# PickNikRobotics/pick_ik

Measured on AMD Instinct MI355X. Metric: converged IK solves/sec (7-DOF Panda, batched random targets), higher is better.
Workload: dtype f64; 1 GPU; panda 7-DOF memetic IK (BASELINE configs[1]): population 128, elites 4, batch 4096 random reachable targets per GPU per step, seed = ready pose, max_generations 100, gd_max_iters 25; robot=panda, dof=7, tip_frames=1, batch_per_gpu=4096, batches_per_call=64, calls=21, streams=4, problems_in_flight_per_gpu=1048576, parallelism=shard1, arithmetic=exact

## Files before the change

### pick_ik_amd/csrc/pik_amd.hip

```cpp
#include <hip/hip_runtime.h>

#include <chrono>
#include <cmath>
#include <cstdlib>
#include <memory>
#include <new>
#include <string>
#include <thread>
#include <vector>

#include "pik_cartesian_ops.hpp"
#include "pik_globalpath_ops.hpp"
#include "pik_interp.hpp"
#include "pik_path_ops.hpp"
#include "pik_polyline_ops.hpp"
#include "pik_restart_ops.hpp"
#include "pik_route_ops.hpp"
#include "pik_search_ops.hpp"
#include "pik_solver.hpp"
#include "pik_startpath_ops.hpp"
#include "pik_urdf.hpp"
#include "pik_pathvalid_ops.hpp"
#include "pik_validity_ops.hpp"

namespace pik {
char* error_buffer() {
    static thread_local char buf[ERROR_BUFFER_SIZE] = "";
    return buf;
}
}

using pik::fail;

#if !defined(PIK_STRICT)
namespace pik_exact {
char* error_buffer() { return ::pik::error_buffer(); }
PIK_DECLARE_OPS_FAMILY(void, launch)
PIK_DECLARE_OPS_FAMILY(void, path)
PIK_DECLARE_OPS_FAMILY(void, search)
PIK_DECLARE_OPS_FAMILY(void, route)
PIK_DECLARE_OPS_FAMILY(void, restart)
PIK_DECLARE_OPS_FAMILY(void, startpath)
PIK_DECLARE_OPS_FAMILY(void, globalpath)
PIK_DECLARE_OPS_FAMILY(void, cartesian)
PIK_DECLARE_OPS_FAMILY(void, polyline)
PIK_DECLARE_OPS_FAMILY(void, validity)
PIK_DECLARE_OPS_FAMILY(void, pathvalid)
}
namespace pik_common {
char* error_buffer() { return ::pik::error_buffer(); }
PIK_DECLARE_OPS_FAMILY(void, launch)
PIK_DECLARE_OPS_FAMILY(void, route)
PIK_DECLARE_OPS_FAMILY(void, restart)
}
namespace pik_common_goals {
char* error_buffer() { return ::pik::error_buffer(); }
PIK_DECLARE_OPS_FAMILY(void, launch)
PIK_DECLARE_OPS_FAMILY(void, route)
PIK_DECLARE_OPS_FAMILY(void, restart)
}
#endif

namespace {

enum Flavour {
    FL_HOME,
#if !defined(PIK_STRICT)
    FL_EXACT,
    FL_COMMON,
    FL_COMMON_GOALS,
#endif
    N_FLAVOURS
};
enum Family { FAM_LAUNCH, FAM_PATH, FAM_SEARCH, FAM_ROUTE, FAM_RESTART, FAM_STARTPATH, FAM_GLOBALPATH, FAM_CARTESIAN, FAM_POLYLINE, FAM_VALIDITY, FAM_PATHVALID, N_FAMILIES };

struct SolverExt : pikamd_solver {
    int search_schedule = pik::SEARCH_ADAPTIVE;
    pik::DevBuf search_rows[pik::N_SLOTS];
    int device_regime = 1;
    long long regime_threshold = 0;
    int routed_passes[pik::N_SLOTS];
    pik::DevBuf restart_rows[pik::N_SLOTS];
    bool gate_set = false;
    pikamd_gate gate = {0.0, 0.0};
    pik::DevBuf gate_params_dev;
    pik::ParamsK gate_params_host[pik::N_SLOTS];
    bool gate_params_valid[pik::N_SLOTS] = {};
    pik::DevBuf startpath_rows[pik::N_SLOTS];
    pik::DevBuf globalpath_rows[pik::N_SLOTS];
    pik::DevBuf cartesian_goals[pik::N_SLOTS];
    pik::DevBuf polyline_rows[pik::N_SLOTS];
    bool validity_set = false;
    pik::ValidityModelK validity_model;
    pik::DevBuf validity_dev;
    uint32_t planar_xy_mask = 0;
    int path_validity = 0;
    pik::DevBuf pathvalid_rows[pik::N_SLOTS];
    SolverExt() {
        for (int& v : routed_passes) v = -1;
    }
};
SolverExt* ext_of(pikamd_solver* s) { return static_cast<SolverExt*>(s); }
const SolverExt* ext_of(const pikamd_solver* s) { return static_cast<const SolverExt*>(s); }

using OpsLookup = const void* (*)(int dof);
template <class Ops, const Ops* (*lookup)(int)>
const void* untyped(int dof) {
    return lookup(dof);
}
const OpsLookup OPS_TABLE[N_FLAVOURS][N_FAMILIES] = {
    {untyped<pik::LaunchOps, pik::launch_ops>, untyped<pik::PathOps, pik::path_ops>, untyped<pik::SearchOps, pik::search_ops>,
#if defined(PIK_STRICT)
     nullptr,
#else
     untyped<pik::RouteOps, pik::route_ops>,
#endif
     untyped<pik::RestartOps, pik::restart_ops>, untyped<pik::StartPathOps, pik::startpath_ops>,
     untyped<pik::GlobalPathOps, pik::globalpath_ops>, untyped<pik::CartesianOps, pik::cartesian_ops>,
     untyped<pik::PolylineOps, pik::polyline_ops>,
#if defined(PIK_STRICT)
     untyped<pik::ValidityOps, pik::validity_ops>, untyped<pik::PathValidOps, pik::pathvalid_ops>},
#else
     nullptr, nullptr},
    {pik_exact::launch_ops, pik_exact::path_ops, pik_exact::search_ops, pik_exact::route_ops, pik_exact::restart_ops,
     pik_exact::startpath_ops, pik_exact::globalpath_ops, pik_exact::cartesian_ops, pik_exact::polyline_ops,
     pik_exact::validity_ops, pik_exact::pathvalid_ops},
    {pik_common::launch_ops, nullptr, nullptr, pik_common::route_ops, pik_common::restart_ops, nullptr, nullptr, nullptr, nullptr, nullptr, nullptr},
    {pik_common_goals::launch_ops, nullptr, nullptr, pik_common_goals::route_ops, pik_common_goals::restart_ops, nullptr, nullptr, nullptr, nullptr, nullptr, nullptr},
#endif
};
const char* const FLAVOUR_NAMESPACE[N_FLAVOURS] = {
#if defined(PIK_STRICT)
    "pik_strict",
#else
    "pik", "pik_exact", "pik_common", "pik_common_goals",
#endif
};

template <class Ops>
const Ops* ops_at(Flavour f, Family family, int dof) {
    const OpsLookup lookup = OPS_TABLE[f][family];
    return lookup ? static_cast<const Ops*>(lookup(dof)) : nullptr;
}

int check_solver(const pikamd_solver* s) {
    if (!s) return fail(PIKAMD_EINVAL, "solver handle is NULL");
    return 0;
}

[[maybe_unused]] bool needs_literal(const pikamd_solver* s) {
    bool f = s->opt.exact || s->chain.float_mask != 0u || s->chain.n_mimic != 0;
    for (int k = 1; k < s->n_tips; ++k) f = f || s->more[k - 1].float_mask != 0u || s->more[k - 1].n_mimic != 0;
    return f;
}
[[maybe_unused]] bool needs_literal(const pikamd_solver* s, const pikamd_params* p) {
    return needs_literal(s) || (p && p->gd_step_size > 1.0e-2);
}

[[maybe_unused]] bool common_eligible(const pikamd_solver* s, const pikamd_params* p, const pik::ParamsK& pk) {
    if (!s->opt.specialised || needs_literal(s)) return false;
    const uint32_t all = (s->chain.dof >= 32) ? ~0u : ((1u << s->chain.dof) - 1u);
    auto chain_ok = [&](const pik::ChainHost& c) {
        return c.prismatic_mask == 0u && c.dh_general_mask == 0u && c.bounded_mask == all;
    };
    if (!chain_ok(s->chain)) return false;
    for (int k = 1; k < s->n_tips; ++k)
        if (!chain_ok(s->more[k - 1])) return false;
    if (pk.line_delta == 0 || !(pk.pos_scale > 0.0) || !(pk.rot_scale > 0.0)) return false;
    if (p->mode == 0 && (pk.elites != 4 || p->memetic_num_threads > 1)) return false;
    return true;
}

Flavour flavour_of(const pikamd_solver* s, const pikamd_params* p, const pik::ParamsK* pk) {
#if defined(PIK_STRICT)
    (void)s, (void)p, (void)pk;
    return FL_HOME;
#else
    if (pk && common_eligible(s, p, *pk)) return pk->goal_mask != 0 ? FL_COMMON_GOALS : FL_COMMON;
    return needs_literal(s, p) ? FL_EXACT : FL_HOME;
#endif
}
bool is_common(Flavour f) {
#if defined(PIK_STRICT)
    (void)f;
    return false;
#else
    return f == FL_COMMON || f == FL_COMMON_GOALS;
#endif
}
Flavour unspecialised(Flavour f) { return is_common(f) ? FL_HOME : f; }
bool is_exact(Flavour f) { return pik::EXACT_FLAVOUR || (f != FL_HOME && !is_common(f)); }

const pik::LaunchOps* ops_of(const pikamd_solver* s, const pikamd_params* p = nullptr) {
    return ops_at<pik::LaunchOps>(flavour_of(s, p, nullptr), FAM_LAUNCH, s->chain.dof);
}
const pik::LaunchOps* solve_ops_of(const pikamd_solver* s, const pikamd_params* p, const pik::ParamsK& pk) {
    const Flavour f = flavour_of(s, p, &pk);
    if (const pik::LaunchOps* o = ops_at<pik::LaunchOps>(f, FAM_LAUNCH, s->chain.dof)) return o;
    return ops_at<pik::LaunchOps>(unspecialised(f), FAM_LAUNCH, s->chain.dof);
}

const pik::RouteOps* route_ops_of(const pikamd_solver* s, const pikamd_params* p, const pik::ParamsK& pk) {
    const pik::SolverOptions& o = s->opt;
    if (!ext_of(s)->device_regime || p->mode != 0 || s->n_tips != 1 || p->memetic_num_threads > 1 || o.lpe != 0 ||
        o.n_sched != 0 || o.regime != 0)
        return nullptr;
    return ops_at<pik::RouteOps>(flavour_of(s, p, &pk), FAM_ROUTE, s->chain.dof);
}

int run_solve(pikamd_solver* s, const pikamd_params* p, const pik::ParamsK& pk, pik::BatchRecord* rec, int n,
              unsigned long long rng_seed, hipStream_t stream, int slot) {
    SolverExt* x = ext_of(s);
    if (const pik::RouteOps* r = route_ops_of(s, p, pk)) {
        pik::RouteCtx ctx;
        ctx.threshold = x->regime_threshold;
        if (int rc = r->solve(s, p, pk, rec, n, rng_seed, stream, slot, &ctx)) return rc;
        if (ctx.served) {
            x->routed_passes[slot] = ctx.n_passes;
            return 0;
        }
    }
    x->routed_passes[slot] = -1;
    return solve_ops_of(s, p, pk)->solve(s, p, pk, rec, n, rng_seed, stream, slot, false);
}

int no_kernels(int dof) {
    return fail(PIKAMD_EUNSUPPORTED, "dof %d: kernels are instantiated for 1..16", dof);
}

const pik::PathOps* path_ops_of(const pikamd_solver* s, const pikamd_params* p) {
    return ops_at<pik::PathOps>(flavour_of(s, p, nullptr), FAM_PATH, s->chain.dof);
}
const pik::SearchOps* search_ops_of(const pikamd_solver* s, const pikamd_params* p) {
    return ops_at<pik::SearchOps>(flavour_of(s, p, nullptr), FAM_SEARCH, s->chain.dof);
}
const pik::StartPathOps* startpath_ops_of(const pikamd_solver* s, const pikamd_params* p) {
    return ops_at<pik::StartPathOps>(flavour_of(s, p, nullptr), FAM_STARTPATH, s->chain.dof);
}
const pik::GlobalPathOps* globalpath_ops_of(const pikamd_solver* s, const pikamd_params* p) {
    return ops_at<pik::GlobalPathOps>(flavour_of(s, p, nullptr), FAM_GLOBALPATH, s->chain.dof);
}
const pik::RestartOps* restart_ops_of(const pikamd_solver* s, const pikamd_params* p, const pik::ParamsK& pk) {
    return ops_at<pik::RestartOps>(flavour_of(s, p, &pk), FAM_RESTART, s->chain.dof);
}

size_t align8(size_t v) { return (v + 7) & ~(size_t)7; }

constexpr size_t GATE_PARAMS_STRIDE = 256;
static_assert(sizeof(pik::ParamsK) <= GATE_PARAMS_STRIDE, "gate parameters slot too small");
int gate_for_call(pikamd_solver* s, const pik::ParamsK& pk, int slot, hipStream_t st, int* on, double* joint,
                  const pik::ParamsK** dev) {
    SolverExt* x = ext_of(s);
    *on = (x->gate_set && pk.approx) ? 1 : 0;
    *joint = x->gate.joint_threshold;
    *dev = nullptr;
    if (!*on) return 0;
    if (int rc = x->gate_params_dev.ensure(GATE_PARAMS_STRIDE * (size_t)pik::N_SLOTS)) return rc;
    char* d = (char*)x->gate_params_dev.p + GATE_PARAMS_STRIDE * (size_t)slot;
    const pik::ParamsK want = pik::gate_params_k(pk, x->gate.cost_threshold);
    if (!x->gate_params_valid[slot] || std::memcmp(&x->gate_params_host[slot], &want, sizeof want) != 0) {
        if (s->consts_valid[slot]) HIP_TRY(hipStreamSynchronize(s->consts_stream[slot]));
        x->gate_params_valid[slot] = false;
        std::memcpy(&x->gate_params_host[slot], &want, sizeof want);
        HIP_TRY(hipMemcpyAsync(d, &x->gate_params_host[slot], sizeof want, hipMemcpyHostToDevice, st));
        HIP_TRY(hipStreamSynchronize(st));
        x->gate_params_valid[slot] = true;
    }
    *dev = reinterpret_cast<const pik::ParamsK*>(d);
    return 0;
}

const pik::ValidityOps* validity_ops_of(const pikamd_solver* s) {
#if defined(PIK_STRICT)
    return ops_at<pik::ValidityOps>(FL_HOME, FAM_VALIDITY, s->chain.dof);
#else
    return ops_at<pik::ValidityOps>(FL_EXACT, FAM_VALIDITY, s->chain.dof);
#endif
}

int validity_chain_ok(const pikamd_solver* s, const char* who) {
    if (s->n_tips != 1) return fail(PIKAMD_EUNSUPPORTED, "%s: the validity model is for handles with one tip frame", who);
    if ((s->chain.float_mask | s->chain.skip_mask) != 0u)
        return fail(PIKAMD_EUNSUPPORTED, "%s: the validity model does not know floating joints", who);
    if (s->chain.n_mimic != 0) return fail(PIKAMD_EUNSUPPORTED, "%s: the validity model does not know mimic joints", who);
    return 0;
}

int validity_for_call(pikamd_solver* s, const char* who, const pik::ValidityOps** ops) {
    *ops = nullptr;
    if (!ext_of(s)->validity_set) return 0;
    if (int rc = validity_chain_ok(s, who)) return rc;
    *ops = validity_ops_of(s);
    return *ops ? 0 : no_kernels(s->chain.dof);
}

int path_validity_for_call(pikamd_solver* s, const char* who, const pik::PathValidOps** ops) {
    *ops = nullptr;
    if (!ext_of(s)->path_validity || !ext_of(s)->validity_set) return 0;
    if (int rc = validity_chain_ok(s, who)) return rc;
#if defined(PIK_STRICT)
    *ops = ops_at<pik::PathValidOps>(FL_HOME, FAM_PATHVALID, s->chain.dof);
#else
    *ops = ops_at<pik::PathValidOps>(FL_EXACT, FAM_PATHVALID, s->chain.dof);
#endif
    return *ops ? 0 : no_kernels(s->chain.dof);
}

int path_validity_reached(pikamd_solver* s, int slot, int64_t P, int32_t* callers, int32_t** out) {
    *out = callers;
    if (callers) return 0;
    pik::DevBuf& buf = ext_of(s)->pathvalid_rows[slot];
// ... 119 lines not shown
    if (int rc = pikamd_urdf_extract(urdf_xml, base_link, tip_links, n_tips, m.get())) return rc;
    if (m->n_tips == 1) {
        const auto& t = m->tips[0];
        pikamd_chain c{m->dof, &t.origin_xyz_rpy[0][0], &t.axis[0][0], t.joint_type, t.tip_xyz_rpy,
                       m->qmin,  m->qmax,               m->vmax,       m->bounded};
        if (int rc = pikamd_create(&c, device_ordinal, out)) return rc;
        if (m->n_mimic)
            if (int rc = pikamd_set_mimic_joints(*out, m->n_mimic, m->mimic)) {
                pikamd_destroy(*out);
                *out = nullptr;
                return rc;
            }
        return 0;
    }
    pikamd_tip tips[PIKAMD_MAX_TIPS];
    for (int k = 0; k < m->n_tips; ++k) {
        const auto& t = m->tips[k];
        tips[k] = pikamd_tip{t.n_joints, t.variable, &t.origin_xyz_rpy[0][0], &t.axis[0][0], t.joint_type, t.tip_xyz_rpy};
    }
    pikamd_multi_chain c{m->dof, m->n_tips, tips, m->qmin, m->qmax, m->vmax, m->bounded};
    if (int rc = pikamd_create_multi(&c, device_ordinal, out)) return rc;
    if (m->n_mimic)
        if (int rc = pikamd_set_mimic_joints(*out, m->n_mimic, m->mimic)) {
            pikamd_destroy(*out);
            *out = nullptr;
            return rc;
        }
    return 0;
}

int32_t pikamd_n_tips(const pikamd_solver* s) { return s ? s->n_tips : 0; }

int32_t pikamd_set_mimic_joints(pikamd_solver* s, int32_t n, const pikamd_mimic_joint* joints) {
    if (int rc = check_solver(s)) return rc;
    if (n < 0 || (n > 0 && !joints)) return fail(PIKAMD_EINVAL, "bad arguments");
    pik::ChainHost saved[PIKAMD_MAX_TIPS];
    for (int k = 0; k < s->n_tips; ++k) saved[k] = k == 0 ? s->chain : s->more[k - 1];
    auto path = [&](int k) -> pik::ChainHost& { return k == 0 ? s->chain : s->more[k - 1]; };
    for (int k = 0; k < s->n_tips; ++k) pik::clear_mimic_joints(path(k));
    for (int i = 0; i < n; ++i) {
        const pikamd_mimic_joint& m = joints[i];
        const char* msg = (m.tip < 0 || m.tip >= s->n_tips) ? "mimic joint: tip out of range" : pik::add_mimic_joint(path(m.tip), m);
        if (!msg && s->n_tips > 1) {
            const uint32_t act = path(m.tip).active_mask;
            if (!((act >> m.master_variable) & 1u) || (m.after_variable >= 0 && !((act >> m.after_variable) & 1u)))
                msg = "mimic joint: master_variable / after_variable is not on that tip's path";
        }
        if (msg) {
            for (int k = 0; k < s->n_tips; ++k) path(k) = saved[k];
            return fail(PIKAMD_EINVAL, "%s", msg);
        }
    }
    s->self_tested.clear();
    s->opt.disabled_lanes = 0;
    s->opt.disabled_lanes_exact = 0;
    return 0;
}

void pikamd_destroy(pikamd_solver* s) {
    if (!s) return;
    (void)hipSetDevice(s->device);
    (void)hipDeviceSynchronize();
    if (s->counters) (void)hipFree(s->counters);
    if (s->consts_dev) (void)hipFree(s->consts_dev);
    if (s->consts_host) (void)hipHostFree(s->consts_host);
    if (s->tables_dev) (void)hipFree(s->tables_dev);
    if (s->tables_host) (void)hipHostFree(s->tables_host);
    for (auto& ev : s->table_event)
        if (ev) (void)hipEventDestroy(ev);
    for (auto& ev : s->slot_event)
        if (ev) (void)hipEventDestroy(ev);
    for (auto& b : s->stage) b.release();
    for (auto& b : s->slot_state) b.release();
    for (auto& b : s->slot_soa) b.release();
    for (auto& b : ext_of(s)->search_rows) b.release();
    for (auto& b : ext_of(s)->restart_rows) b.release();
    for (auto& b : ext_of(s)->startpath_rows) b.release();
    for (auto& b : ext_of(s)->cartesian_goals) b.release();
    for (auto& b : ext_of(s)->polyline_rows) b.release();
    for (auto& b : ext_of(s)->globalpath_rows) b.release();
    ext_of(s)->gate_params_dev.release();
    ext_of(s)->validity_dev.release();
    for (auto& b : ext_of(s)->pathvalid_rows) b.release();
    for (auto& j : s->jobs) {
        j.dev.release();
        j.host.release();
        if (j.stream) (void)hipStreamDestroy(j.stream);
    }
    delete ext_of(s);
}

int32_t pikamd_variables(const pikamd_solver* s, double* out) {
    if (int rc = check_solver(s)) return rc;
    if (!out) return fail(PIKAMD_EINVAL, "out is NULL");
    for (int j = 0; j < s->chain.dof; ++j) {
        out[7 * j + 0] = s->chain.qmin[j];
        out[7 * j + 1] = s->chain.qmax[j];
        out[7 * j + 2] = s->chain.mid[j];
        out[7 * j + 3] = s->chain.hspan[j];
        out[7 * j + 4] = s->chain.vrcp[j];
        out[7 * j + 5] = s->chain.mdf[j];
        out[7 * j + 6] = ((s->chain.bounded_mask >> j) & 1u) ? 1.0 : 0.0;
    }
    return 0;
}

int32_t pikamd_fk_batch_device(pikamd_solver* s, int64_t n, const double* d_q, double* d_pos_quat,
                               void* stream) {
    if (int rc = check_solver(s)) return rc;
    if (n < 0 || (n > 0 && (!d_q || !d_pos_quat))) return fail(PIKAMD_EINVAL, "bad arguments");
    HIP_TRY(hipSetDevice(s->device));
    return ops_of(s)->fk(s, n, d_q, d_pos_quat, (hipStream_t)stream);
}

int32_t pikamd_fk_batch(pikamd_solver* s, int64_t n, const double* q, double* pos_quat) {
    if (int rc = check_solver(s)) return rc;
    if (n < 0 || (n > 0 && (!q || !pos_quat))) return fail(PIKAMD_EINVAL, "bad arguments");
    if (n == 0) return 0;
    HIP_TRY(hipSetDevice(s->device));
    const size_t d = (size_t)s->chain.dof;
    if (int rc = s->stage[0].ensure(sizeof(double) * d * (size_t)n)) return rc;
    if (int rc = s->stage[1].ensure(sizeof(double) * 7 * (size_t)s->n_tips * (size_t)n)) return rc;
    HIP_TRY(hipMemcpy(s->stage[0].p, q, sizeof(double) * d * (size_t)n, hipMemcpyHostToDevice));
    if (int rc = pikamd_fk_batch_device(s, n, (const double*)s->stage[0].p, (double*)s->stage[1].p, nullptr))
        return rc;
    HIP_TRY(hipMemcpy(pos_quat, s->stage[1].p, sizeof(double) * 7 * (size_t)s->n_tips * (size_t)n, hipMemcpyDeviceToHost));
    return 0;
}

int32_t pikamd_cost_batch(pikamd_solver* s, const pikamd_params* p, int64_t n,
                          const double* goal_pos_quat, const double* seed, const double* q,
                          double* cost, int32_t* is_solution) {
    if (int rc = check_solver(s)) return rc;
    pik::ParamsK pk;
    if (!p) return fail(PIKAMD_EINVAL, "params is NULL");
    if (const char* msg = pik::make_params_k(p, pk)) {
        pikamd_params q2 = *p;
        q2.mode = 1;
        if (const char* m2 = pik::make_params_k(&q2, pk)) return fail(PIKAMD_EINVAL, "%s", m2);
        (void)msg;
    }
    if (n < 0 || (n > 0 && (!goal_pos_quat || !seed || !q))) return fail(PIKAMD_EINVAL, "bad arguments");
    if (n == 0) return 0;
    HIP_TRY(hipSetDevice(s->device));
    const size_t d = (size_t)s->chain.dof, N = (size_t)n;
    if (int rc = s->stage[0].ensure(sizeof(double) * 7 * (size_t)s->n_tips * N)) return rc;
    if (int rc = s->stage[1].ensure(sizeof(double) * d * N)) return rc;
    if (int rc = s->stage[2].ensure(sizeof(double) * d * N)) return rc;
    if (int rc = s->stage[3].ensure(sizeof(double) * N)) return rc;
    if (int rc = s->stage[4].ensure(sizeof(int) * N)) return rc;
    HIP_TRY(hipMemcpy(s->stage[0].p, goal_pos_quat, sizeof(double) * 7 * (size_t)s->n_tips * N, hipMemcpyHostToDevice));
    HIP_TRY(hipMemcpy(s->stage[1].p, seed, sizeof(double) * d * N, hipMemcpyHostToDevice));
    HIP_TRY(hipMemcpy(s->stage[2].p, q, sizeof(double) * d * N, hipMemcpyHostToDevice));
    if (int rc = ops_of(s)->cost(s, pk, n, (const double*)s->stage[0].p, (const double*)s->stage[1].p,
                                 (const double*)s->stage[2].p, cost ? (double*)s->stage[3].p : nullptr,
                                 is_solution ? (int*)s->stage[4].p : nullptr, nullptr))
        return rc;
    if (cost) HIP_TRY(hipMemcpy(cost, s->stage[3].p, sizeof(double) * N, hipMemcpyDeviceToHost));
    if (is_solution) HIP_TRY(hipMemcpy(is_solution, s->stage[4].p, sizeof(int) * N, hipMemcpyDeviceToHost));
    HIP_TRY(hipDeviceSynchronize());
    return 0;
}

int32_t pikamd_gd_step_batch(pikamd_solver* s, const pikamd_params* p, int64_t n,
                             const double* goal_pos_quat, const double* seed, double* local,
                             double* best, double* local_cost, double* best_cost,
// ... 62 lines not shown
        r.stats = b.stats;
        r.completed = b.completed;
        sum += b.B;
    }
    (void)s;
    *total = sum;
    return n;
}

__global__ void pik_joint_layout_kernel(const double* __restrict__ in, double* __restrict__ out, long long B, int D,
                                        int to_aos) {
    const long long i = (long long)blockIdx.x * blockDim.x + threadIdx.x;
    if (i >= B * D) return;
    if (to_aos) {
        const long long b = i / D;
        const int j = (int)(i - b * D);
        out[i] = in[(long long)j * B + b];
    } else {
        const long long j = i / B, b = i - j * B;
        out[i] = in[b * D + j];
    }
}

static int maybe_self_test(pikamd_solver* s, const pikamd_params* p);

static int32_t solve_records(pikamd_solver* s, const pikamd_params* p, pik::BatchRecord* rec, int n,
                             uint64_t rng_seed, hipStream_t stream, int slot) {
    pik::ParamsK pk;
    if (const char* msg = pik::make_params_k(p, pk)) return fail(PIKAMD_EINVAL, "%s", msg);
    if (n == 0) return 0;
    HIP_TRY(hipSetDevice(s->device));
    if (!s->opt.soa) return run_solve(s, p, pk, rec, n, rng_seed, stream, slot);
    const int D = s->chain.dof;
    size_t doubles = 0;
    for (int k = 0; k < n; ++k) {
        if (rec[k].completed)
            return fail(PIKAMD_EINVAL, "joint_layout soa: completion counters are not available (the solutions of a "
                                       "batch are in place when the stream has passed the call)");
        doubles += (size_t)rec[k].B * (size_t)D * (rec[k].guess != rec[k].seed ? 3u : 2u);
    }
    if (int rc = s->slot_soa[slot].ensure(sizeof(double) * doubles)) return rc;
    double* w = (double*)s->slot_soa[slot].p;
    double* user_solution[PIKAMD_MAX_BATCHES];
    auto move = [&](const double* in, double* out, long long B, int to_aos) -> int {
        const long long items = B * D;
        hipLaunchKernelGGL(pik_joint_layout_kernel, dim3((unsigned)((items + 255) / 256)), dim3(256), 0, stream, in, out, B,
                           D, to_aos);
        HIP_TRY(hipGetLastError());
        return 0;
    };
    for (int k = 0; k < n; ++k) {
        const long long B = rec[k].B;
        const bool own_guess = rec[k].guess != rec[k].seed;
        double* sd = w;
        w += (size_t)B * D;
        if (int rc = move(rec[k].seed, sd, B, 1)) return rc;
        double* gs = sd;
        if (own_guess) {
            gs = w;
            w += (size_t)B * D;
            if (int rc = move(rec[k].guess, gs, B, 1)) return rc;
        }
        user_solution[k] = rec[k].solution;
        rec[k].seed = sd;
        rec[k].guess = gs;
        rec[k].solution = w;
        w += (size_t)B * D;
    }
    if (int rc = run_solve(s, p, pk, rec, n, rng_seed, stream, slot)) return rc;
    for (int k = 0; k < n; ++k)
        if (int rc = move(rec[k].solution, user_solution[k], rec[k].B, 0)) return rc;
    return 0;
}

int32_t pikamd_solve_batches_device(pikamd_solver* s, const pikamd_params* p, int32_t n_batches,
                                    const pikamd_batch* batches, uint64_t rng_seed, void* stream,
                                    int32_t slot) {
    if (int rc = check_solver(s)) return rc;
    if (slot < 0 || slot >= PIKAMD_MAX_SLOTS) return fail(PIKAMD_EINVAL, "slot out of range");
    pik::BatchRecord rec[PIKAMD_MAX_BATCHES];
    long long total = 0;
    const int n = make_records(s, n_batches, batches, rec, &total);
    if (n < 0) return n;
    return solve_records(s, p, rec, n, rng_seed, (hipStream_t)stream, slot);
}

int32_t pikamd_solve_batch_device(pikamd_solver* s, const pikamd_params* p, int64_t B,
                                  const double* d_goal_pos_quat, const double* d_seed,
                                  uint64_t rng_seed, int64_t problem_offset, double* d_solution,
                                  int32_t* d_status, double* d_final_cost, pikamd_stats* d_stats,
                                  void* stream, int32_t slot) {
    const pikamd_batch b = {B,          d_goal_pos_quat, d_seed,       nullptr, problem_offset,
                            d_solution, d_status,        d_final_cost, d_stats, nullptr};
    return pikamd_solve_batches_device(s, p, 1, &b, rng_seed, stream, slot);
}

int32_t pikamd_reserve(pikamd_solver* s, const pikamd_params* p, int64_t B, int32_t slot, void* stream) {
    if (int rc = check_solver(s)) return rc;
    pik::ParamsK pk;
    if (const char* msg = pik::make_params_k(p, pk)) return fail(PIKAMD_EINVAL, "%s", msg);
    if (B < 0) return fail(PIKAMD_EINVAL, "bad arguments");
    if (slot < 0 || slot >= PIKAMD_MAX_SLOTS) return fail(PIKAMD_EINVAL, "slot out of range");
    if (B == 0) return 0;
    if (int rc = maybe_self_test(s, p)) return rc;
    HIP_TRY(hipSetDevice(s->device));
    if (s->opt.soa)
        if (int rc = s->slot_soa[slot].ensure(sizeof(double) * (size_t)B * (size_t)s->chain.dof * 3u)) return rc;
    pik::BatchRecord rec;
    std::memset(&rec, 0, sizeof rec);
    rec.B = B;
    return solve_ops_of(s, p, pk)->solve(s, p, pk, &rec, 1, 0, (hipStream_t)stream, slot, true);
}

static int32_t start_job(pikamd_solver* s, const pikamd_params* p, int32_t n_batches,
                         const pikamd_batch* batches, uint64_t rng_seed, int job) {
    if (int rc = check_solver(s)) return rc;
    if (job < 0 || job > pik::JOB_SELF_TEST) return fail(PIKAMD_EINVAL, "job out of range");
    if (job != pik::JOB_SELF_TEST)
        if (int rc = maybe_self_test(s, p)) return rc;
    pik::HostJob& J = s->jobs[job];
    if (J.pending) return fail(PIKAMD_EINVAL, "job %d is still in flight: call pikamd_wait first", job);
    pik::BatchRecord rec[PIKAMD_MAX_BATCHES];
    long long total = 0;
    const int n = make_records(s, n_batches, batches, rec, &total);
    if (n < 0) return n;
    {
        pik::ParamsK pk;
        if (const char* msg = pik::make_params_k(p, pk)) return fail(PIKAMD_EINVAL, "%s", msg);
    }
    J.n_batches = 0;
    if (n == 0) return 0;
    HIP_TRY(hipSetDevice(s->device));
    if (!J.stream) HIP_TRY(hipStreamCreateWithFlags(&J.stream, hipStreamNonBlocking));
    const size_t d = (size_t)s->chain.dof, g7 = 7 * (size_t)s->n_tips;
    size_t off = 0;
    size_t in_goal[PIKAMD_MAX_BATCHES], in_seed[PIKAMD_MAX_BATCHES], in_guess[PIKAMD_MAX_BATCHES];
    for (int k = 0; k < n; ++k) {
        const size_t N = (size_t)rec[k].B;
        in_goal[k] = off;
        off += sizeof(double) * g7 * N;
        in_seed[k] = off;
        off += sizeof(double) * d * N;
        in_guess[k] = (rec[k].guess != rec[k].seed) ? off : in_seed[k];
        if (rec[k].guess != rec[k].seed) off += sizeof(double) * d * N;
    }
    J.in_bytes = off;
    for (int k = 0; k < n; ++k) {
        const size_t N = (size_t)rec[k].B;
        pik::HostJob::Out& o = J.outs[k];
        o.B = rec[k].B;
        o.solution = rec[k].solution;
        o.status = rec[k].status;
        o.final_cost = rec[k].cost;
        o.stats = (pikamd_stats*)rec[k].stats;
        o.off_solution = off;
        off += sizeof(double) * d * N;
        o.off_cost = off;
        off += sizeof(double) * N;
        o.off_stats = off;
        off += sizeof(pikamd_stats) * N;
        o.off_status = off;
        off += align8(sizeof(int32_t) * N);
    }
    J.out_bytes = off - J.in_bytes;
    if (int rc = J.dev.ensure(off)) return rc;
    if (int rc = J.host.ensure(off)) return rc;
    char* hb = (char*)J.host.p;
    char* db = (char*)J.dev.p;
    for (int k = 0; k < n; ++k) {
        const size_t N = (size_t)rec[k].B;
        std::memcpy(hb + in_goal[k], rec[k].goal, sizeof(double) * g7 * N);
        std::memcpy(hb + in_seed[k], rec[k].seed, sizeof(double) * d * N);
        if (in_guess[k] != in_seed[k]) std::memcpy(hb + in_guess[k], rec[k].guess, sizeof(double) * d * N);
        rec[k].goal = (const double*)(db + in_goal[k]);
        rec[k].seed = (const double*)(db + in_seed[k]);
        rec[k].guess = (const double*)(db + in_guess[k]);
        rec[k].solution = (double*)(db + J.outs[k].off_solution);
        rec[k].status = (int*)(db + J.outs[k].off_status);
        rec[k].cost = (double*)(db + J.outs[k].off_cost);
        rec[k].stats = (void*)(db + J.outs[k].off_stats);
        rec[k].completed = nullptr;
    }
    HIP_TRY(hipMemcpyAsync(db, hb, J.in_bytes, hipMemcpyHostToDevice, J.stream));
    if (int rc = solve_records(s, p, rec, n, rng_seed, J.stream, pik::N_DEVICE_SLOTS + job)) {
        (void)hipStreamSynchronize(J.stream);
        return rc;
    }
    {
// ... 119 lines not shown
        if (v != "none" && (!ints(v, ',', x) || x.size() > 15))
            return fail(PIKAMD_EINVAL, "passes: expected 'none' or up to 15 ascending generation marks, got '%s'", v.c_str());
        for (size_t k = 0; k < x.size(); ++k)
            if (x[k] <= 0 || (k > 0 && x[k] <= x[k - 1]))
                return fail(PIKAMD_EINVAL, "passes: marks must be positive and ascending, got '%s'", v.c_str());
        o.passes_set = true;
        o.n_marks = (int)x.size();
        for (size_t k = 0; k < x.size(); ++k) o.marks[k] = x[k];
        return 0;
    }
    if (n == "two_per_simd") {
        if (v.empty()) { o.two_per_simd = -1; return 0; }
        std::vector<int> x;
        if (!ints(v, ',', x) || x.size() != 1 || x[0] < 0)
            return fail(PIKAMD_EINVAL, "two_per_simd: expected 0, 1 or a wavefront threshold, got '%s'", v.c_str());
        o.two_per_simd = x[0];
        return 0;
    }
    if (n == "arithmetic") {
#if defined(PIK_STRICT)
        if (v.empty() || v == "exact") return 0;
        return fail(PIKAMD_EINVAL, "arithmetic: the verification library only has 'exact', got '%s'", v.c_str());
#else
        if (v.empty() || v == "exact") { o.exact = true; return 0; }
        if (v == "fast") { o.exact = false; return 0; }
        return fail(PIKAMD_EINVAL, "arithmetic: expected 'fast' or 'exact', got '%s'", v.c_str());
#endif
    }
    if (n == "self_test") {
        if (v.empty() || v == "auto") { o.auto_self_test = true; return 0; }
        if (v == "off") { o.auto_self_test = false; return 0; }
        return fail(PIKAMD_EINVAL, "self_test: expected 'auto' or 'off', got '%s'", v.c_str());
    }
    if (n == "specialised") {
        if (v.empty() || v == "1") { o.specialised = true; return 0; }
        if (v == "0") { o.specialised = false; return 0; }
        return fail(PIKAMD_EINVAL, "specialised: expected '0' or '1', got '%s'", v.c_str());
    }
    if (n == "shard_chunks") {
        if (v.empty()) { o.shard_chunks = 0; return 0; }
        std::vector<int> x;
        if (!ints(v, ',', x) || x.size() != 1 || x[0] < 1 || x[0] > 8)
            return fail(PIKAMD_EINVAL, "shard_chunks: expected 1..8, got '%s'", v.c_str());
        o.shard_chunks = x[0];
        return 0;
    }
    if (n == "joint_layout") {
        if (v.empty() || v == "aos") { o.soa = false; return 0; }
        if (v == "soa") { o.soa = true; return 0; }
        return fail(PIKAMD_EINVAL, "joint_layout: expected 'aos' or 'soa', got '%s'", v.c_str());
    }
    if (n == "host_max_time" || n == "host_gd_max_time") {
        double x = 0.0;
        if (!v.empty()) {
            char* end = nullptr;
            x = std::strtod(v.c_str(), &end);
            if (end == v.c_str() || *end != 0 || !(x >= 0.0) || !std::isfinite(x))
                return fail(PIKAMD_EINVAL, "%s: expected a time in seconds >= 0, got '%s'", n.c_str(), v.c_str());
        }
        (n == "host_max_time" ? o.host_max_time : o.host_gd_max_time) = x;
        return 0;
    }
    if (n == "search_schedule") {
        int& sched = ext_of(s)->search_schedule;
        if (v.empty() || v == "adaptive") { sched = pik::SEARCH_ADAPTIVE; return 0; }
        if (v == "sequential") { sched = pik::SEARCH_SEQUENTIAL; return 0; }
        if (v == "parallel") { sched = pik::SEARCH_PARALLEL; return 0; }
        return fail(PIKAMD_EINVAL, "search_schedule: expected 'adaptive', 'sequential' or 'parallel', got '%s'", v.c_str());
    }
    if (n == "device_regime") {
        int x = 1;
        if (!pik::parse_device_regime(v.c_str(), &x))
            return fail(PIKAMD_EINVAL, "device_regime: expected '0' or '1', got '%s'", v.c_str());
        ext_of(s)->device_regime = x;
        return 0;
    }
    if (n == "regime_threshold") {
        if (v.empty()) { ext_of(s)->regime_threshold = 0; return 0; }
        std::vector<int> x;
        if (!ints(v, ',', x) || x.size() != 1 || x[0] < 0)
            return fail(PIKAMD_EINVAL, "regime_threshold: expected a number of problems >= 0, got '%s'", v.c_str());
        ext_of(s)->regime_threshold = x[0];
        return 0;
    }
    if (n == "regime") {
        if (v.empty() || v == "adaptive") { o.regime = 0; return 0; }
        if (v == "latency") { o.regime = 1; return 0; }
        if (v == "throughput") { o.regime = 2; return 0; }
        return fail(PIKAMD_EINVAL, "regime: expected 'adaptive', 'latency' or 'throughput', got '%s'", v.c_str());
    }
    return fail(PIKAMD_EINVAL, "unknown option '%s'", n.c_str());
}


void pikamd_shard_bounds(int64_t total, int32_t rank, int32_t world, int64_t* lo, int64_t* hi) {
    if (world < 1) world = 1;
    if (total < 0) total = 0;
    const int64_t base = total / world, rem = total % world;
    const int64_t l = (int64_t)rank * base + (rank < rem ? rank : rem);
    if (lo) *lo = l;
    if (hi) *hi = l + base + (rank < rem ? 1 : 0);
}

int32_t pikamd_solve_batch_sharded(pikamd_solver* const* solvers, int32_t n_devices, const pikamd_params* p,
                                   int64_t B, const double* goal_pos_quat, const double* seed,
                                   const double* initial_guess, uint64_t rng_seed, int64_t problem_offset,
                                   double* solution, int32_t* status, double* final_cost, pikamd_stats* stats) {
    if (!solvers || n_devices < 1) return fail(PIKAMD_EINVAL, "no solver handles");
    if (B < 0 || (B > 0 && (!goal_pos_quat || !seed || !solution || !status))) return fail(PIKAMD_EINVAL, "bad arguments");
    for (int r = 0; r < n_devices; ++r) {
        if (!solvers[r]) return fail(PIKAMD_EINVAL, "solver handle %d is NULL", r);
        if (solvers[r]->chain.dof != solvers[0]->chain.dof || solvers[r]->n_tips != solvers[0]->n_tips)
            return fail(PIKAMD_EINVAL, "solver handle %d describes a different chain", r);
        for (int q = 0; q < r; ++q)
            if (solvers[q] == solvers[r]) return fail(PIKAMD_EINVAL, "solver handle %d is given twice", r);
    }
    if (B == 0) return 0;
    for (int r = 0; r < n_devices; ++r)
        if (solvers[r]->opt.soa)
            return fail(PIKAMD_EINVAL, "joint_layout soa: not with pikamd_solve_batch_sharded (a shard of a [dof][B] "
                                       "array is not contiguous)");
    const size_t d = (size_t)solvers[0]->chain.dof, g7 = 7 * (size_t)solvers[0]->n_tips;
    constexpr int MAX_CHUNKS = 2;
    constexpr int64_t CHUNK_MIN = 32768;
    std::vector<int> rc((size_t)n_devices, 0);
    std::vector<std::string> msg((size_t)n_devices);
    auto work = [&](int r) {
        int64_t lo = 0, hi = 0;
        pikamd_shard_bounds(B, r, n_devices, &lo, &hi);
        const int64_t n = hi - lo;
        if (n == 0) return;
        int chunks = (int)((n + CHUNK_MIN - 1) / CHUNK_MIN);
        const int max_chunks = solvers[r]->opt.shard_chunks > 0 ? solvers[r]->opt.shard_chunks : MAX_CHUNKS;
        chunks = chunks < 1 ? 1 : chunks > max_chunks ? max_chunks : chunks;
        int started = 0;
        for (int c = 0; c < chunks && rc[r] == 0; ++c) {
            int64_t clo = 0, chi = 0;
            pikamd_shard_bounds(n, c, chunks, &clo, &chi);
            const int64_t a = lo + clo;
            const pikamd_batch b = {chi - clo,
                                    goal_pos_quat + (size_t)a * g7,
                                    seed + (size_t)a * d,
                                    initial_guess ? initial_guess + (size_t)a * d : nullptr,
                                    problem_offset + a,
                                    solution + (size_t)a * d,
                                    status + a,
                                    final_cost ? final_cost + a : nullptr,
                                    stats ? stats + a : nullptr,
                                    nullptr};
            rc[r] = pikamd_solve_batches_async(solvers[r], p, 1, &b, rng_seed, c);
            if (rc[r] == 0) ++started;
        }
        for (int c = 0; c < started; ++c) {
            const int w = pikamd_wait(solvers[r], c);
            if (rc[r] == 0) rc[r] = w;
        }
        if (rc[r] != 0) msg[r] = pik::error_buffer();
    };
    if (n_devices == 1) {
        work(0);
    } else {
        std::vector<std::thread> th;
        th.reserve((size_t)n_devices);
        for (int r = 0; r < n_devices; ++r) th.emplace_back(work, r);
        for (auto& t : th) t.join();
    }
    for (int r = 0; r < n_devices; ++r)
        if (rc[r] != 0) return fail(rc[r], "device shard %d: %s", r, msg[r].c_str());
    return 0;
}

#if defined(PIK_STRICT)
#define PIK_HOST_SOLVE pik_strict_host_solve
#else
#define PIK_HOST_SOLVE pik_exact_host_solve
#endif
}
extern "C" int PIK_HOST_SOLVE(const pikamd_solver* s, const pikamd_params* p, long long B, const double* goal,
                              const double* seed, const double* guess, unsigned long long rng_seed,
                              long long problem_offset, pikamd_cost_fn cb, void* user, double* solution, int32_t* status,
                              double* final_cost, pikamd_stats* stats);
extern "C" {

int32_t pikamd_solve_batch_host(pikamd_solver* s, const pikamd_params* p, int64_t B, const double* goal_pos_quat,
                                const double* seed, const double* initial_guess, uint64_t rng_seed,
                                int64_t problem_offset, pikamd_cost_fn cost_fn, void* user, double* solution,
                                int32_t* status, double* final_cost, pikamd_stats* stats) {
    if (int rc = check_solver(s)) return rc;
    if (!p) return fail(PIKAMD_EINVAL, "params is NULL");
    if (!cost_fn)
        return fail(PIKAMD_EINVAL, "pikamd_solve_batch_host is for queries with a host cost function; without one "
                                   "use pikamd_solve_batch (the GPU)");
    if (B < 0 || (B > 0 && (!goal_pos_quat || !seed || !solution || !status))) return fail(PIKAMD_EINVAL, "bad arguments");
    if (p->mode == 0 && (p->memetic_elite_size < 1 || p->memetic_population_size <= p->memetic_elite_size))
        return fail(PIKAMD_EINVAL, "memetic_population_size must exceed memetic_elite_size >= 1");
    if (s->opt.soa)
        return fail(PIKAMD_EINVAL, "joint_layout soa: not with pikamd_solve_batch_host (its arrays are [B][dof])");
    return PIK_HOST_SOLVE(s, p, B, goal_pos_quat, seed, initial_guess, rng_seed, problem_offset, cost_fn, user, solution,
                          status, final_cost, stats);
}

int32_t pikamd_self_test(pikamd_solver* s, const pikamd_params* p, int32_t n, uint32_t* disabled_out) {
    if (int rc = check_solver(s)) return rc;
    if (!p) return fail(PIKAMD_EINVAL, "params is NULL");
    if (n < 1 || n > 4096) return fail(PIKAMD_EINVAL, "n out of range [1, 4096]");
    const bool exact_now = is_exact(flavour_of(s, p, nullptr));
    auto mask_of = [exact_now](pik::SolverOptions& o) -> unsigned& { return exact_now ? o.disabled_lanes_exact : o.disabled_lanes; };
    if (disabled_out) *disabled_out = mask_of(s->opt);
    const int d = s->chain.dof, tips = s->n_tips;
    std::vector<double> q((size_t)n * d), goal((size_t)n * 7 * tips), seed((size_t)n * d);
    unsigned long long x = 0x9E3779B97F4A7C15ull;
    for (int i = 0; i < n; ++i)
        for (int j = 0; j < d; ++j) {
            x = x * 6364136223846793005ull + 1442695040888963407ull;
            const double u = (double)(x >> 11) * (1.0 / 9007199254740992.0);
            const bool bounded = (s->chain.bounded_mask >> j) & 1u;
            const double lo = bounded ? s->chain.qmin[j] : -3.0, hi = bounded ? s->chain.qmax[j] : 3.0;
            q[(size_t)i * d + j] = lo + (hi - lo) * u;
            seed[(size_t)i * d + j] = bounded ? 0.5 * (lo + hi) : 0.0;
        }
    if (int rc = pikamd_fk_batch(s, n, q.data(), goal.data())) return rc;
    struct Out {
        std::vector<double> sol, cost;
        std::vector<int32_t> st;
        std::vector<pikamd_stats> stats;
    };
    pik::SolverOptions saved = s->opt;
    auto run = [&](int lanes, bool passes, bool occ2, Out& o) -> int {
        s->opt = saved;
        s->opt.soa = false;
        s->opt.lpe = lanes;
        s->opt.n_sched = 0;
        s->opt.passes_set = true;
        s->opt.n_marks = 0;
        if (passes) {
            const int m[] = {1, 2, 3, 4, 7, 11, 16, 24, 40, 64};
            for (int v : m) s->opt.marks[s->opt.n_marks++] = v;
        }
        s->opt.two_per_simd = occ2 ? 1 : 0;
        s->opt.force_occ2 = occ2;
        s->opt.regime = 1;
        o.sol.assign((size_t)n * d, 0.0);
        o.cost.assign((size_t)n, 0.0);
        o.st.assign((size_t)n, 0);
        o.stats.assign((size_t)n, pikamd_stats{});
        const pikamd_batch b = {n,            goal.data(), seed.data(),   nullptr,        0,
                                o.sol.data(), o.st.data(), o.cost.data(), o.stats.data(), nullptr};
        int rc = start_job(s, p, 1, &b, 12345, pik::JOB_SELF_TEST);
        if (!rc) rc = wait_job(s, pik::JOB_SELF_TEST);
        s->opt = saved;
        return rc;
    };
    auto same = [&](const Out& a, const Out& b) {
        return std::memcmp(a.sol.data(), b.sol.data(), sizeof(double) * a.sol.size()) == 0 &&
               std::memcmp(a.cost.data(), b.cost.data(), sizeof(double) * a.cost.size()) == 0 &&
               std::memcmp(a.st.data(), b.st.data(), sizeof(int32_t) * a.st.size()) == 0 &&
               std::memcmp(a.stats.data(), b.stats.data(), sizeof(pikamd_stats) * a.stats.size()) == 0;
    };
    const bool multi = tips > 1;
    const int S = (p->mode == 0 && p->memetic_num_threads > 1) ? p->memetic_num_threads : 1;
    int gs = 1;
    while (p->mode == 0 && gs < p->memetic_elite_size) gs <<= 1;
    auto served = [&](int lanes) -> bool {
        if (mask_of(saved) & (unsigned)lanes) return false;
        return pik::lpe_allowed(s, lanes, gs, S, multi, exact_now);
    };
    Out ref, got;
    unsigned disabled = 0;
    if (p->mode != 0) {
        if (int rc = run(1, false, false, ref)) return rc;
#if !defined(PIK_STRICT)
        if (!needs_literal(s) && !exact_now)
            for (int lanes : {8, 16}) {
                if (!served(lanes)) continue;
                if (int rc = run(lanes, false, false, got)) return rc;
                if (!same(ref, got)) disabled |= (unsigned)lanes;
            }
#endif
        if (exact_now && !multi)
            for (int lanes : {4, 16}) {
                if (!served(lanes)) continue;
                if (int rc = run(lanes, false, false, got)) return rc;
                if (!same(ref, got)) disabled |= (unsigned)lanes;
            }
        mask_of(s->opt) = mask_of(saved) | disabled;
        if (disabled_out) *disabled_out = mask_of(s->opt);
        return 0;
    }
    if (int rc = run(1, false, false, ref)) return rc;
    for (int lanes : {2, 4, 8, 16}) {
        if (!served(lanes)) continue;
        for (int passes = 0; passes < 2; ++passes) {
            if (int rc = run(lanes, passes != 0, false, got)) return rc;
            if (!same(ref, got)) disabled |= (unsigned)lanes;
        }
    }
    {
        pik::ParamsK pk;
        if (!pik::make_params_k(p, pk) && is_common(flavour_of(s, p, &pk))) {
            const bool was = s->opt.specialised;
            s->opt.specialised = false;
            Out general;
            saved.specialised = false;
            const int rc = run(1, false, false, general);
            saved.specialised = was;
            s->opt.specialised = was;
            if (rc) return rc;
            if (!same(ref, general)) disabled |= 32u;
        }
    }
// ... 1333 lines not shown
```

### pick_ik_amd/solver.py

```python
from __future__ import annotations

import ctypes as C
import os

import numpy as np

_HERE = os.path.dirname(os.path.abspath(__file__))
LIB_PATH = os.environ.get("PIK_LIB") or os.path.join(_HERE, "libpick_ik_amd.so")
LIB_STRICT_PATH = os.environ.get("PIK_LIB_STRICT") or os.path.join(_HERE, "libpick_ik_amd_strict.so")

SUCCESS = 1
APPROXIMATE = 2
NO_IK_SOLUTION = -31
NOT_ATTEMPTED = 0
PATH_JUMP = -1001
MAX_ATTEMPTS = 64
MAX_SLOTS = 128
MAX_BATCHES = 64
MAX_HOST_JOBS = 16


class PickIkAmdError(RuntimeError):
    pass

# ... 399 lines not shown
        h = C.c_void_p()
        lim = [_f64(chain.qmin), _f64(chain.qmax), _f64(chain.vmax),
               np.ascontiguousarray(chain.bounded, dtype=np.uint8)]
        if hasattr(chain, "tips"):
            keep, tips = [lim], (_Tip * self.n_tips)()
            for i, t in enumerate(chain.tips):
                a = [np.ascontiguousarray(t.variable, dtype=np.int32), _f64(t.origin_xyz_rpy),
                     _f64(t.axis), np.ascontiguousarray(t.joint_type, dtype=np.int32),
                     _f64(t.tip_xyz_rpy)]
                keep.append(a)
                tips[i] = _Tip(len(a[0]), _ip(a[0]), _dp(a[1]), _dp(a[2]), _ip(a[3]), _dp(a[4]))
            self._keep = (keep, tips)
            c = _MultiChain(self.dof, self.n_tips, tips, _dp(lim[0]), _dp(lim[1]), _dp(lim[2]),
                            lim[3].ctypes.data_as(C.POINTER(C.c_uint8)))
            self._chk(self._L.pikamd_create_multi(C.byref(c), self.device, C.byref(h)))
        else:
            k = [_f64(chain.origin_xyz_rpy), _f64(chain.axis),
                 np.ascontiguousarray(chain.joint_type, dtype=np.int32), _f64(chain.tip_xyz_rpy)]
            self._keep = (k, lim)
            c = _Chain(self.dof, _dp(k[0]), _dp(k[1]), _ip(k[2]), _dp(k[3]), _dp(lim[0]),
                       _dp(lim[1]), _dp(lim[2]), lim[3].ctypes.data_as(C.POINTER(C.c_uint8)))
            self._chk(self._L.pikamd_create(C.byref(c), self.device, C.byref(h)))
        self._h = h
        arr = mimic_array(chain)
        if arr is not None:
            self._chk(self._L.pikamd_set_mimic_joints(self._h, len(arr), arr))
        if not self.strict and exact is not None:
            self.set_option("arithmetic", "exact" if exact else "fast")
        self._env_options()

    @classmethod
    def from_urdf(cls, urdf: str, base_link: str, tip_links, device: int = 0, strict: bool = False):
        chain, names = urdf_extract(urdf, base_link, tip_links, strict)
        self = cls.__new__(cls)
        self._L = lib(strict)
        self.strict, self.chain, self.variable_names = strict, chain, names
        self.exact = not strict
        self.dof, self.device, self.n_tips = int(chain.dof), int(device), int(getattr(chain, "n_tips", 1))
        tips = [tip_links] if isinstance(tip_links, str) else list(tip_links)
        arr = (C.c_char_p * len(tips))(*[t.encode() for t in tips])
        h = C.c_void_p()
        self._keep = None
        _check(self._L.pikamd_create_from_urdf(_urdf_text(urdf), base_link.encode(), arr, len(tips), self.device,
                                               C.byref(h)), self._L)
        self._h = h
        return self

    def _chk(self, rc: int):
        _check(rc, self._L)

    def set_option(self, name: str, value) -> None:
        v = b"" if value is None else str(value).encode()
        self._chk(self._L.pikamd_set_option(self._h, name.encode(), v))

    VARIANT_LANES = {5: 16, 4: 8, 3: 4, 2: 2, 1: 1, 7: 1}
    MAX_PASSES = 16

    def debug_regime(self, slot: int = 0, publish_load: int = -1):
        n = C.c_int32(0)
        sv = np.zeros(self.MAX_PASSES, dtype=np.uint32)
        ol = np.zeros(self.MAX_PASSES, dtype=np.uint32)
        var = np.zeros(self.MAX_PASSES, dtype=np.int32)
        up = C.POINTER(C.c_uint32)
        self._chk(self._L.pikamd_debug_regime(self._h, slot, int(publish_load), self.MAX_PASSES, C.byref(n),
                                              sv.ctypes.data_as(up), ol.ctypes.data_as(up), _ip(var)))
        if n.value < 0:
            return None
        return [(int(sv[k]), int(ol[k]), int(var[k])) for k in range(n.value)]

    def self_test(self, params: Params, n: int = 64) -> int:
        m = C.c_uint32(0)
        self._chk(self._L.pikamd_self_test(self._h, C.byref(params), n, C.byref(m)))
        return int(m.value)

    def self_test_cost(self):
        runs, ms = C.c_int32(0), C.c_double(0.0)
        self._chk(self._L.pikamd_self_test_cost(self._h, C.byref(runs), C.byref(ms)))
        return int(runs.value), float(ms.value)

    ENV_OPTIONS = (("PIK_LPE", "lanes_per_elite"), ("PIK_LPE_SCHED", "lanes_per_elite_schedule"),
                   ("PIK_PASSES", "passes"), ("PIK_OCC2", "two_per_simd"), ("PIK_REGIME", "regime"),
                   ("PIK_SPECIALISED", "specialised"), ("PIK_SHARD_CHUNKS", "shard_chunks"),
                   ("PIK_SELF_TEST", "self_test"), ("PIK_DEVICE_REGIME", "device_regime"),
                   ("PIK_REGIME_THRESHOLD", "regime_threshold"))

    def _env_options(self) -> None:
        cur = tuple(os.environ.get(k) for k, _ in self.ENV_OPTIONS)
        seen = getattr(self, "_env_seen", (None,) * len(cur))
        if cur == seen:
            return
        for (_, name), new, old in zip(self.ENV_OPTIONS, cur, seen):
            if new != old:
                self.set_option(name, new)
        self._env_seen = cur

    def close(self):
        if getattr(self, "_h", None):
            self._L.pikamd_destroy(self._h)
            self._h = None

    def __del__(self):
        try:
            self.close()
        except Exception:
            pass

    def variables(self) -> np.ndarray:
        out = np.empty((self.dof, 7))
        self._chk(self._L.pikamd_variables(self._h, _dp(out)))
        return out

    def fk(self, q) -> np.ndarray:
        q = _f64(q).reshape(-1, self.dof)
        out = np.empty((q.shape[0], 7) if self.n_tips == 1 else (q.shape[0], self.n_tips, 7))
        self._chk(self._L.pikamd_fk_batch(self._h, q.shape[0], _dp(q), _dp(out)))
        return out

    def cost(self, params: Params, goal_pos_quat, seed, q):
        q = _f64(q).reshape(-1, self.dof)
        n = q.shape[0]
        g7 = 7 * self.n_tips
        goal = np.ascontiguousarray(np.broadcast_to(_f64(goal_pos_quat).reshape(-1, g7), (n, g7)))
        seed = np.ascontiguousarray(np.broadcast_to(_f64(seed).reshape(-1, self.dof),
                                                    (n, self.dof)))
        cost = np.empty(n)
        sol = np.empty(n, dtype=np.int32)
        self._chk(self._L.pikamd_cost_batch(self._h, C.byref(params), n, _dp(goal), _dp(seed), _dp(q),
                                       _dp(cost), _ip(sol)))
        return cost, sol

    def gate(self, params: Params, gate: Gate, goal_pos_quat, seed, q) -> np.ndarray:
        q = _f64(q).reshape(-1, self.dof)
        n = q.shape[0]
        g7 = 7 * self.n_tips
        goal = np.ascontiguousarray(np.broadcast_to(_f64(goal_pos_quat).reshape(-1, g7), (n, g7)))
        seed = np.ascontiguousarray(np.broadcast_to(_f64(seed).reshape(-1, self.dof), (n, self.dof)))
        ok = np.zeros(n, dtype=np.int32)
        self._chk(self._L.pikamd_gate_batch(self._h, C.byref(params), C.byref(gate), n, _dp(goal), _dp(seed), _dp(q),
                                            _ip(ok)))
        return ok != 0

    def set_approximate_gate(self, cost_threshold: float = 0.0, joint_threshold: float = 0.0) -> None:
        self._chk(self._L.pikamd_set_approximate_gate(self._h, C.byref(Gate(cost_threshold, joint_threshold))))

    def clear_approximate_gate(self) -> None:
        self._chk(self._L.pikamd_set_approximate_gate(self._h, None))

    def set_validity_model(self, spheres, pairs) -> None:
        sph = [s if isinstance(s, Sphere) else Sphere(*s) for s in spheres]
        arr = (Sphere * max(1, len(sph)))(*sph)
        pr = np.ascontiguousarray(np.asarray(pairs, dtype=np.int32).reshape(-1, 2))
        m = ValidityModel(len(sph), arr, pr.shape[0], pr.ctypes.data_as(C.POINTER(C.c_int32)))
        self._chk(self._L.pikamd_set_validity_model(self._h, C.byref(m)))
        self._n_spheres = len(sph)

    def clear_validity_model(self) -> None:
        self._chk(self._L.pikamd_set_validity_model(self._h, None))
        self._n_spheres = None

    def set_path_validity(self, on: bool) -> None:
        self._chk(self._L.pikamd_set_path_validity(self._h, 1 if on else 0))

    def validity(self, q, centres: bool = False):
        q = _f64(q).reshape(-1, self.dof)
        n = q.shape[0]
        ns = getattr(self, "_n_spheres", None) or 0
        valid = np.zeros(n, dtype=np.int32)
# ... 490 lines not shown
```

Measured before the change: 3.009 million solves/s.

## Fork per-slot device solves onto private streams joined back to caller

Gives each device slot its own non-blocking HIP stream. A device solve forks onto that stream with an event and joins back to the caller's stream with a second event. The default mode turns this on once more than one slot has been seen, so that solves issued on the same caller stream from different slots can run concurrently on the GPU. This costs extra event record/wait overhead per call and more stream objects, and capture mode falls back to the caller stream. It also drops the self-test stream afterwards.

```diff
diff --git a/pick_ik_amd/csrc/pik_amd.hip b/pick_ik_amd/csrc/pik_amd.hip
--- a/pick_ik_amd/csrc/pik_amd.hip
+++ b/pick_ik_amd/csrc/pik_amd.hip
@@ -96,6 +96,11 @@
     uint32_t planar_xy_mask = 0;
     int path_validity = 0;
     pik::DevBuf pathvalid_rows[pik::N_SLOTS];
+    int slot_streams = -1;
+    hipStream_t slot_stream[pik::N_DEVICE_SLOTS] = {};
+    hipEvent_t slot_fork[pik::N_DEVICE_SLOTS] = {}, slot_join[pik::N_DEVICE_SLOTS] = {};
+    bool slot_seen[pik::N_DEVICE_SLOTS] = {};
+    int n_slots_seen = 0;
     SolverExt() {
         for (int& v : routed_passes) v = -1;
     }
@@ -227,6 +232,62 @@
 int no_kernels(int dof) {
     return fail(PIKAMD_EUNSUPPORTED, "dof %d: kernels are instantiated for 1..16", dof);
 }
+
+bool slot_streams_wanted(const SolverExt* x) {
+    return x->slot_streams == 1 || (x->slot_streams < 0 && x->n_slots_seen > 1);
+}
+
+int slot_streams_prepare(pikamd_solver* s, int slot) {
+    SolverExt* x = ext_of(s);
+    if (!x->slot_seen[slot]) {
+        x->slot_seen[slot] = true;
+        ++x->n_slots_seen;
+    }
+    if (!slot_streams_wanted(x)) return 0;
+    for (int k = 0; k < pik::N_DEVICE_SLOTS; ++k) {
+        if (!x->slot_seen[k] || x->slot_stream[k]) continue;
+        if (!x->slot_fork[k]) HIP_TRY(hipEventCreateWithFlags(&x->slot_fork[k], hipEventDisableTiming));
+        if (!x->slot_join[k]) HIP_TRY(hipEventCreateWithFlags(&x->slot_join[k], hipEventDisableTiming));
+        HIP_TRY(hipStreamCreateWithFlags(&x->slot_stream[k], hipStreamNonBlocking));
+    }
+    return 0;
+}
+
+struct SlotFork {
+    pikamd_solver* s;
+    int slot;
+    hipStream_t caller;
+    bool forked = false;
+    SlotFork(pikamd_solver* s_, int slot_, hipStream_t caller_) : s(s_), slot(slot_), caller(caller_) {}
+    int begin(hipStream_t* st) {
+        *st = caller;
+        SolverExt* x = ext_of(s);
+        HIP_TRY(hipSetDevice(s->device));
+        hipStreamCaptureStatus cap = hipStreamCaptureStatusNone;
+        if (hipStreamIsCapturing(caller, &cap) != hipSuccess || cap != hipStreamCaptureStatusNone) {
+            (void)hipGetLastError();
+            return 0;
+        }
+        if (int rc = slot_streams_prepare(s, slot)) return rc;
+        if (!slot_streams_wanted(x)) return 0;
+        HIP_TRY(hipEventRecord(x->slot_fork[slot], caller));
+        HIP_TRY(hipStreamWaitEvent(x->slot_stream[slot], x->slot_fork[slot], 0));
+        forked = true;
+        *st = x->slot_stream[slot];
+        return 0;
+    }
+    int end(int launch_rc) {
+        if (!forked) return launch_rc;
+        SolverExt* x = ext_of(s);
+        hipError_t e = hipEventRecord(x->slot_join[slot], x->slot_stream[slot]);
+        if (e == hipSuccess) e = hipStreamWaitEvent(caller, x->slot_join[slot], 0);
+        if (e != hipSuccess) {
+            (void)hipStreamSynchronize(x->slot_stream[slot]);
+            if (!launch_rc) return fail(PIKAMD_EHIP, "slot %d: joining the caller's stream failed: %s", slot, hipGetErrorString(e));
+        }
+        return launch_rc;
+    }
+};
 
 const pik::PathOps* path_ops_of(const pikamd_solver* s, const pikamd_params* p) {
     return ops_at<pik::PathOps>(flavour_of(s, p, nullptr), FAM_PATH, s->chain.dof);
@@ -512,6 +573,12 @@
     ext_of(s)->gate_params_dev.release();
     ext_of(s)->validity_dev.release();
     for (auto& b : ext_of(s)->pathvalid_rows) b.release();
+    for (auto& st : ext_of(s)->slot_stream)
+        if (st) (void)hipStreamDestroy(st);
+    for (auto& ev : ext_of(s)->slot_fork)
+        if (ev) (void)hipEventDestroy(ev);
+    for (auto& ev : ext_of(s)->slot_join)
+        if (ev) (void)hipEventDestroy(ev);
     for (auto& j : s->jobs) {
         j.dev.release();
         j.host.release();
@@ -740,7 +807,11 @@
     long long total = 0;
     const int n = make_records(s, n_batches, batches, rec, &total);
     if (n < 0) return n;
-    return solve_records(s, p, rec, n, rng_seed, (hipStream_t)stream, slot);
+    if (n == 0) return solve_records(s, p, rec, n, rng_seed, (hipStream_t)stream, slot);
+    SlotFork fork(s, slot, (hipStream_t)stream);
+    hipStream_t st = nullptr;
+    if (int rc = fork.begin(&st)) return rc;
+    return fork.end(solve_records(s, p, rec, n, rng_seed, st, slot));
 }
 
 int32_t pikamd_solve_batch_device(pikamd_solver* s, const pikamd_params* p, int64_t B,
@@ -762,6 +833,7 @@
     if (B == 0) return 0;
     if (int rc = maybe_self_test(s, p)) return rc;
     HIP_TRY(hipSetDevice(s->device));
+    if (int rc = slot_streams_prepare(s, slot)) return rc;
     if (s->opt.soa)
         if (int rc = s->slot_soa[slot].ensure(sizeof(double) * (size_t)B * (size_t)s->chain.dof * 3u)) return rc;
     pik::BatchRecord rec;
@@ -1047,6 +1119,11 @@
             return fail(PIKAMD_EINVAL, "regime_threshold: expected a number of problems >= 0, got '%s'", v.c_str());
         ext_of(s)->regime_threshold = x[0];
         return 0;
+    }
+    if (n == "slot_streams") {
+        if (v.empty() || v == "auto") { ext_of(s)->slot_streams = -1; return 0; }
+        if (v == "0" || v == "1") { ext_of(s)->slot_streams = v == "1" ? 1 : 0; return 0; }
+        return fail(PIKAMD_EINVAL, "slot_streams: expected 'auto', '0' or '1', got '%s'", v.c_str());
     }
     if (n == "regime") {
         if (v.empty() || v == "adaptive") { o.regime = 0; return 0; }
@@ -1191,6 +1268,16 @@
         std::vector<pikamd_stats> stats;
     };
     pik::SolverOptions saved = s->opt;
+    struct DropStream {
+        pikamd_solver* s;
+        ~DropStream() {
+            pik::HostJob& j = s->jobs[pik::JOB_SELF_TEST];
+            if (j.stream) (void)hipStreamDestroy(j.stream);
+            j.stream = nullptr;
+            s->consts_valid[pik::N_DEVICE_SLOTS + pik::JOB_SELF_TEST] = false;
+            s->consts_stream[pik::N_DEVICE_SLOTS + pik::JOB_SELF_TEST] = nullptr;
+        }
+    } drop_stream{s};
     auto run = [&](int lanes, bool passes, bool occ2, Out& o) -> int {
         s->opt = saved;
         s->opt.soa = false;
diff --git a/pick_ik_amd/solver.py b/pick_ik_amd/solver.py
--- a/pick_ik_amd/solver.py
+++ b/pick_ik_amd/solver.py
@@ -505,7 +505,7 @@
                    ("PIK_PASSES", "passes"), ("PIK_OCC2", "two_per_simd"), ("PIK_REGIME", "regime"),
                    ("PIK_SPECIALISED", "specialised"), ("PIK_SHARD_CHUNKS", "shard_chunks"),
                    ("PIK_SELF_TEST", "self_test"), ("PIK_DEVICE_REGIME", "device_regime"),
-                   ("PIK_REGIME_THRESHOLD", "regime_threshold"))
+                   ("PIK_REGIME_THRESHOLD", "regime_threshold"), ("PIK_SLOT_STREAMS", "slot_streams"))
 
     def _env_options(self) -> None:
         cur = tuple(os.environ.get(k) for k, _ in self.ENV_OPTIONS)
```

After: 2.705 million solves/s. -10.1%, worse.
